# akanazawa/human_dynamics

Measured on NVIDIA H100. Metric: frames/sec (ResNet->f_movie->SMPL LBS), higher is better.
Workload: dtype f32 (wgmma 3x fp16 head/remainder split, fp32 two-level accumulate)

## Files before the change

human_dynamics_b200/csrc/conv_tc.cu:

```cuda
#include <cuda.h>
#include <cuda_fp16.h>
#include <cstdlib>
#include "conv_common.cuh"
#include "tc_ptx.cuh"

namespace hd {
namespace {

constexpr int BM = 128;
constexpr int A_TILE_BYTES = BM * 128;
constexpr int BOX_BYTES = 64 * 128;
constexpr int W_PROD = 8;
constexpr int STAGE_OUT = 1, STAGE_PAIR = 2;

using namespace ptx;

template <bool HALF, bool ASPLIT, int BN, bool RES = false>
struct Cfg {
  static_assert(BN == 64 || (BN == 128 && HALF && ASPLIT), "128-wide N tiles: pre-split fp16 path only");
  static_assert(!RES || ASPLIT, "residual by TMA: pre-split fp16 path only");
  static constexpr int PROD_THREADS = BN == 128 ? 128 : 256;
  static constexpr int NUM_THREADS = 256 + PROD_THREADS;
  static constexpr int ROW_STEP = PROD_THREADS / 8;
  static constexpr int ROWS = BM / ROW_STEP;
  static constexpr int PROD_REGS = BN == 128 ? 40 : 104, CONS_REGS = BN == 128 ? 232 : 152;
  static_assert(256 * CONS_REGS + PROD_THREADS * PROD_REGS <= 65536, "setmaxnreg split beyond the register file");
  static constexpr int NACC = BN / 2;
  static constexpr int STAGES = BN == 128 ? (RES ? 2 : 3) : (RES ? 3 : 4);
  static constexpr int BKE = HALF ? 64 : 32;
  static constexpr int B_TILE_BYTES = BN * 128;
  static constexpr int STAGE_BYTES = 2 * A_TILE_BYTES + 2 * B_TILE_BYTES;
  static constexpr int RES_OFFSET = STAGES * STAGE_BYTES;
  static constexpr int RES_SLOT_BYTES = RES ? 64 * BN * 4 : 0;
  static constexpr int STG_OFFSET = RES_OFFSET + 2 * RES_SLOT_BYTES;
  static constexpr int STG_BYTES = ASPLIT ? 2 * BOX_BYTES : 0;
  static constexpr int BAR_OFFSET = STG_OFFSET + 2 * STG_BYTES;
  static constexpr int SMEM_BYTES = BAR_OFFSET + 128 + 1024;
  static_assert(SMEM_BYTES <= 232448, "dynamic shared memory beyond the 227 KB a CTA can opt into");
  static constexpr int PF = HALF ? 2 : 3;
  static constexpr int V = HALF ? 2 : 1;
};

template <int R>
struct RowState {
  int n[R], iy[R], ix[R];
};

template <bool SPLIT, int PCH, bool HALF, bool GATHER, bool ASPLIT, int BN, bool RES>
__global__ void __launch_bounds__((Cfg<HALF, ASPLIT, BN, RES>::NUM_THREADS), 1)
conv_gemm_tc_kernel(const ConvParams p, const __grid_constant__ CUtensorMap tmap_hi, const __grid_constant__ CUtensorMap tmap_lo,
                    const __grid_constant__ CUtensorMap tmap_res, const __grid_constant__ CUtensorMap tmap_out,
                    const __grid_constant__ CUtensorMap tmap_out_hi, const __grid_constant__ CUtensorMap tmap_out_lo, const int stage) {
  using C = Cfg<HALF, ASPLIT, BN, RES>;
  constexpr int BKE = C::BKE, PF = C::PF, V = C::V, STAGES = C::STAGES, R = C::ROWS, RS = C::ROW_STEP, NA = C::NACC;
  extern __shared__ uint8_t smem_raw[];
  const uint32_t smem_base = (smem_u32(smem_raw) + 1023u) & ~1023u;
  uint8_t *smem = smem_raw + (smem_base - smem_u32(smem_raw));
  const uint32_t bar_base = smem_base + C::BAR_OFFSET;
  auto full_bar = [&](int s) { return bar_base + 8u * s; };
  auto empty_bar = [&](int s) { return bar_base + 8u * (STAGES + s); };
  auto res_bar = [&](int g) { return bar_base + 8u * (2 * STAGES + g); };

  const int warp = threadIdx.x >> 5, lane = threadIdx.x & 31;
  const int num_k = (GATHER ? p.K_pad : p.K) / BKE;
  const int tiles_n = (p.Cout + BN - 1) / BN;
  const int num_tiles = ((p.M + BM - 1) / BM) * tiles_n;
  const int my_tiles = (num_tiles - (int)blockIdx.x + (int)gridDim.x - 1) / (int)gridDim.x;

  if (threadIdx.x == 0) {
    for (int s = 0; s < STAGES; ++s) {
      mbar_init(full_bar(s), ASPLIT ? C::PROD_THREADS + 1 : 9);
      mbar_init(empty_bar(s), 8);
    }
    if (RES) for (int g = 0; g < 2; ++g) mbar_init(res_bar(g), 1);
    asm volatile("fence.mbarrier_init.release.cluster;" ::: "memory");
  }
  __syncthreads();
  const int xmode = p.dbg ? (int)p.dbg[15] : 0;

  if (warp >= W_PROD) {
    asm volatile("setmaxnreg.dec.sync.aligned.u32 %0;" ::"n"(C::PROD_REGS));
    const int t = threadIdx.x - W_PROD * 32;
    const int j = t & 7;
    const int rb = t >> 3;
    const uint32_t sw_off = (uint32_t)((j ^ (rb & 7)) << 4);
    const bool prof = p.dbg != nullptr && blockIdx.x == 0 && t == 0;
    long long t_wait = 0, t_start = prof && BN == 64 ? clock64() : 0;
    if (BN == 128 && prof) p.dbg[0] = clock64();
    const int total = my_tiles * num_k;
    auto load_b = [&](int s, int ti, int kc) {
      if (t != 0) return;
      const int n0 = (((int)blockIdx.x + ti * (int)gridDim.x) % tiles_n) * BN;
      const uint32_t b_hi = smem_base + s * C::STAGE_BYTES + 2 * A_TILE_BYTES;
      if (xmode & 2) { mbar_arrive(full_bar(s)); return; }
      const int boxes = (BN == 128 && n0 + 64 < p.Cout) ? 2 : 1;
      mbar_arrive_expect_tx(full_bar(s), (SPLIT ? 2 : 1) * boxes * BOX_BYTES);
      for (int b = 0; b < boxes; ++b) {
        tma_load_2d(b_hi + b * BOX_BYTES, &tmap_hi, full_bar(s), kc * BKE, n0 + 64 * b);
        if (SPLIT) tma_load_2d(b_hi + C::B_TILE_BYTES + b * BOX_BYTES, &tmap_lo, full_bar(s), kc * BKE, n0 + 64 * b);
      }
    };

    auto enter_tile = [&](int ti, RowState<R> &rs) {
      const int tile = (int)blockIdx.x + ti * (int)gridDim.x;
      const int m0 = (tile / tiles_n) * BM;
      const int hw = p.Ho * p.Wo;
#pragma unroll
      for (int i = 0; i < R; ++i) {
        const int m = m0 + rb + RS * i;
        if (m < p.M) {
          const int n = m / hw;
          const int r = m - n * hw;
          const int oy = r / p.Wo, ox = r - oy * p.Wo;
          rs.n[i] = n; rs.iy[i] = oy * p.stride - p.pad_t; rs.ix[i] = ox * p.stride - p.pad_l;
        } else {
          rs.n[i] = -1; rs.iy[i] = 0; rs.ix[i] = 0;
        }
      }
    };
    if constexpr (ASPLIT) {
      const __half *ihi = reinterpret_cast<const __half *>(p.in_hi);
      const __half *ilo = reinterpret_cast<const __half *>(p.in_lo);
      if (!p.planes && p.KH * p.KW <= 32 && (long long)p.n_img * p.H * p.W * p.in_ld < (1ll << 31)) {
        const uint32_t off0 = (uint32_t)rb * 128u + sw_off;
        int base[R];
        uint32_t mask[R];
        int kc = 0, ti = 0, tap = 0, ci0 = 0, kx = 0, ky = 0, tap_off = 0;
        for (int q = 0; q < total; ++q) {
          if (kc == 0) {
            const int tile = (int)blockIdx.x + ti * (int)gridDim.x;
            const int m0 = (tile / tiles_n) * BM + rb;
            const int hw = p.Ho * p.Wo;
#pragma unroll
            for (int i = 0; i < R; ++i) {
              const int m = m0 + RS * i;
              uint32_t mk = 0;
              int b = 0;
              if (m < p.M) {
                const int n = m / hw;
                const int r = m - n * hw;
                const int oy = r / p.Wo, ox = r - oy * p.Wo;
                const int iy0 = oy * p.stride - p.pad_t, ix0 = ox * p.stride - p.pad_l;
                b = ((n * p.H + iy0) * p.W + ix0) * p.in_ld + j * 8;
                int t = 0;
                for (int yy = 0; yy < p.KH; ++yy)
                  for (int xx = 0; xx < p.KW; ++xx, ++t)
                    if ((unsigned)(iy0 + yy) < (unsigned)p.H && (unsigned)(ix0 + xx) < (unsigned)p.W) mk |= 1u << t;
              }
              base[i] = b;
              mask[i] = mk;
            }
            tap = 0; ci0 = 0; kx = 0; ky = 0; tap_off = 0;
          }
          const int s = q % STAGES;
          const uint32_t ph = (uint32_t)(q / STAGES) & 1u;
          long long tw0 = prof ? clock64() : 0;
          mbar_wait(empty_bar(s), ph ^ 1u);
          if (prof) t_wait += clock64() - tw0;
          load_b(s, ti, kc);
          const uint32_t a_hi = smem_base + s * C::STAGE_BYTES + off0;
          const int eo = tap_off + ci0;
#pragma unroll
          for (int i = 0; i < R; ++i) {
            const bool ok = (mask[i] >> tap) & 1u;
            const int e = ok ? base[i] + eo : 0;
            cp_async16(a_hi + i * RS * 128, ihi + e, ok ? 16u : 0u);
            cp_async16(a_hi + A_TILE_BYTES + i * RS * 128, ilo + e, ok ? 16u : 0u);
          }
          asm volatile("cp.async.mbarrier.arrive.noinc.shared::cta.b64 [%0];" ::"r"(full_bar(s)) : "memory");
          ci0 += BKE;
          if (ci0 == p.Cin) {
            ci0 = 0; ++tap;
            if (++kx == p.KW) { kx = 0; ++ky; }
            tap_off = (ky * p.W + kx) * p.in_ld;
          }
          if (++kc == num_k) { kc = 0; ++ti; }
        }
      } else if (p.planes && (long long)p.n_img * p.H * p.W * p.in_ld < (1ll << 31)) {
        const uint32_t off0 = (uint32_t)rb * 128u + sw_off;
        const int jt = j >> 2;
        const int row_step = 2 * p.W * (int)p.in_ld;
        int base[R];
        int kc = 0, ti = 0;
        for (int q = 0; q < total; ++q) {
          if (kc == 0) {
            const int tile = (int)blockIdx.x + ti * (int)gridDim.x;
            const int m0 = (tile / tiles_n) * BM + rb;
            const int hw = p.Ho * p.Wo;
#pragma unroll
            for (int i = 0; i < R; ++i) {
              const int m = m0 + RS * i;
              int b = -1;
              if (m < p.M) {
                const int n = m / hw;
                const int r = m - n * hw;
                const int oy = r / p.Wo, ox = r - oy * p.Wo;
                b = ((n * p.H + oy * p.stride + jt) * p.W + ox * p.stride) * (int)p.in_ld + (j & 3) * 8;
              }
              base[i] = b;
            }
          }
          const int s = q % STAGES;
          const uint32_t ph = (uint32_t)(q / STAGES) & 1u;
          long long tw0 = prof ? clock64() : 0;
          mbar_wait(empty_bar(s), ph ^ 1u);
          if (prof) t_wait += clock64() - tw0;
          load_b(s, ti, kc);
          const uint32_t a_hi = smem_base + s * C::STAGE_BYTES + off0;
          const bool tap_ok = 2 * kc + jt < 7;
          const int eo = kc * row_step;
#pragma unroll
          for (int i = 0; i < R; ++i) {
            const bool ok = tap_ok && base[i] >= 0;
            const int e = ok ? base[i] + eo : 0;
            cp_async16_ca(a_hi + i * RS * 128, ihi + e, ok ? 16u : 0u);
            cp_async16_ca(a_hi + A_TILE_BYTES + i * RS * 128, ilo + e, ok ? 16u : 0u);
          }
          asm volatile("cp.async.mbarrier.arrive.noinc.shared::cta.b64 [%0];" ::"r"(full_bar(s)) : "memory");
          if (++kc == num_k) { kc = 0; ++ti; }
        }
      } else {
      RowState<R> rs;
      int kc = 0, ti = 0;
      for (int q = 0; q < total; ++q) {
        if (kc == 0) enter_tile(ti, rs);
        const int s = q % STAGES;
        const uint32_t ph = (uint32_t)(q / STAGES) & 1u;
        long long tw0 = prof ? clock64() : 0;
        mbar_wait(empty_bar(s), ph ^ 1u);
        if (prof) t_wait += clock64() - tw0;
        load_b(s, ti, kc);
        const int kb = kc * BKE;
        const int tap = p.planes ? 2 * kc + (j >> 2) : kb / p.Cin;
        const int ci = p.planes ? (j & 3) * 8 : kb - tap * p.Cin + j * 8;
        const int ky = tap / p.KW, kx = tap - ky * p.KW;
        const bool tap_ok = !p.planes || tap < 7;
        const uint32_t a_hi = smem_base + s * C::STAGE_BYTES, a_lo = a_hi + A_TILE_BYTES;
#pragma unroll
        for (int i = 0; i < R; ++i) {
          const int iy = rs.iy[i] + ky, ix = rs.ix[i] + kx;
          const bool ok = tap_ok && rs.n[i] >= 0 && iy >= 0 && iy < p.H && ix >= 0 && ix < p.W;
          const size_t e = ok ? ((size_t)((size_t)rs.n[i] * p.H + iy) * p.W + ix) * p.in_ld + ci : 0;
          const uint32_t off = (uint32_t)(rb + RS * i) * 128u + sw_off;
          if (p.planes) {
            cp_async16_ca(a_hi + off, ihi + e, ok ? 16u : 0u);
            cp_async16_ca(a_lo + off, ilo + e, ok ? 16u : 0u);
          } else {
            cp_async16(a_hi + off, ihi + e, ok ? 16u : 0u);
            cp_async16(a_lo + off, ilo + e, ok ? 16u : 0u);
          }
        }
        asm volatile("cp.async.mbarrier.arrive.noinc.shared::cta.b64 [%0];" ::"r"(full_bar(s)) : "memory");
        if (++kc == num_k) { kc = 0; ++ti; }
      }
      }
      cp_async_commit();
      cp_async_wait<0>();
      if (prof) { p.dbg[0] = clock64() - (BN == 128 ? p.dbg[0] : t_start); p.dbg[1] = t_wait; }
    } else {
    RowState<R> pf_rs, st_rs;
    float4 ring[PF][4 * V];
    uint32_t vmask[PF];
    int pf_kc = 0, pf_ti = 0;
    auto prefetch = [&](float4 *dst, uint32_t &vm) {
      if (pf_kc == 0) enter_tile(pf_ti, pf_rs);
      if (GATHER) {
        const int seg = p.KW * p.Cin, segp = (seg + 7) & ~7;
        const int g8 = (pf_kc * BKE + j * (4 * V)) / 8;
        const int gpr = segp >> 3;
        const int ky = g8 / gpr, r0 = (g8 - ky * gpr) * 8;
        vm = 0;
#pragma unroll
        for (int i = 0; i < 4; ++i) {
          const int iy = pf_rs.iy[i] + ky;
          const bool okr = pf_rs.n[i] >= 0 && ky < p.KH && iy >= 0 && iy < p.H;
          const int c0 = pf_rs.ix[i] * p.Cin + r0;
          const float *src = p.in + ((size_t)((size_t)(okr ? pf_rs.n[i] : 0) * p.H + (okr ? iy : 0)) * p.W) * p.in_ld + c0;
          const int rowlen = p.W * p.Cin;
          float xs[8];
#pragma unroll
          for (int e = 0; e < 8; ++e) {
            const bool ok = okr && (r0 + e) < seg && (c0 + e) >= 0 && (c0 + e) < rowlen;
            xs[e] = ok ? __ldg(src + e) : 0.f;
          }
          dst[i * V] = make_float4(xs[0], xs[1], xs[2], xs[3]);
          dst[i * V + V - 1] = make_float4(xs[4], xs[5], xs[6], xs[7]);
          if (pf_rs.n[i] >= 0) vm |= 1u << i;
        }
        if (++pf_kc == num_k) { pf_kc = 0; ++pf_ti; }
        return;
      }
      const int kb = pf_kc * BKE;
      const int tap = kb / p.Cin, ci = kb - tap * p.Cin + j * (4 * V);
      const int ky = tap / p.KW, kx = tap - ky * p.KW;
      vm = 0;
#pragma unroll
      for (int i = 0; i < 4; ++i) {
        const int iy = pf_rs.iy[i] + ky, ix = pf_rs.ix[i] + kx;
        const bool ok = pf_rs.n[i] >= 0 && iy >= 0 && iy < p.H && ix >= 0 && ix < p.W;
        if (ok && !(xmode & 4)) {
          const float4 *src = reinterpret_cast<const float4 *>(p.in + ((size_t)((size_t)pf_rs.n[i] * p.H + iy) * p.W + ix) * p.in_ld + ci);
#pragma unroll
          for (int v = 0; v < V; ++v) dst[i * V + v] = __ldg(src + v);
          vm |= 1u << i;
        } else {
#pragma unroll
          for (int v = 0; v < V; ++v) dst[i * V + v] = make_float4(0.f, 0.f, 0.f, 0.f);
        }
      }
      if (++pf_kc == num_k) { pf_kc = 0; ++pf_ti; }
    };
// ... 22 lines not shown
#pragma unroll
          for (int v = 0; v < V; ++v) {
            const float4 sc = __ldg(reinterpret_cast<const float4 *>(p.pre_scale + po) + v);
            const float4 sh = __ldg(reinterpret_cast<const float4 *>(p.pre_shift + po) + v);
            xs[4 * v] = xs[4 * v] * sc.x + sh.x; xs[4 * v + 1] = xs[4 * v + 1] * sc.y + sh.y;
            xs[4 * v + 2] = xs[4 * v + 2] * sc.z + sh.z; xs[4 * v + 3] = xs[4 * v + 3] * sc.w + sh.w;
          }
          if (p.pre_relu) {
#pragma unroll
            for (int e = 0; e < 4 * V; ++e) xs[e] = fmaxf(xs[e], 0.f);
          }
        }
        uint32_t h[4], l[4];
        if (!HALF) {
#pragma unroll
          for (int e = 0; e < 4; ++e) {
            const float hf = rn_tf32(xs[e]);
            h[e] = __float_as_uint(hf);
            l[e] = __float_as_uint(rn_tf32(xs[e] - hf));
          }
        } else {
#pragma unroll
          for (int e = 0; e < 4; ++e) split_f16x2(xs[2 * e], xs[2 * e + 1], h[e], l[e]);
        }
        const uint32_t off = (uint32_t)(rb + 32 * i) * 128u + sw_off;
        if (xmode & 1) continue;
        *reinterpret_cast<uint4 *>(a_hi + off) = make_uint4(h[0], h[1], h[2], h[3]);
        if (SPLIT) *reinterpret_cast<uint4 *>(a_lo + off) = make_uint4(l[0], l[1], l[2], l[3]);
      }
      asm volatile("fence.proxy.async.shared::cta;" ::: "memory");
      __syncwarp();
      if (lane == 0) mbar_arrive(full_bar(s));
      if (++st_kc == num_k) { st_kc = 0; ++st_ti; }
    };
#pragma unroll
    for (int u = 0; u < PF - 1; ++u)
      if (u < total) prefetch(ring[u], vmask[u]);
    for (int q0 = 0; q0 < total; q0 += PF) {
#pragma unroll
      for (int u = 0; u < PF; ++u) {
        const int q = q0 + u;
        if (q < total) {
          if (q + PF - 1 < total) prefetch(ring[(u + PF - 1) % PF], vmask[(u + PF - 1) % PF]);
          consume(q, ring[u], vmask[u]);
        }
      }
    }
    if (prof) { p.dbg[0] = clock64() - t_start; p.dbg[1] = t_wait; }
    }
  } else if (warp < W_PROD) {
    asm volatile("setmaxnreg.inc.sync.aligned.u32 %0;" ::"n"(C::CONS_REGS));
    const int wg = warp >> 2;
    const bool prof = p.dbg != nullptr && blockIdx.x == 0 && threadIdx.x == 0;
    long long t_wait = 0, t_start = prof && BN == 64 && !RES ? clock64() : 0;
    if ((RES || BN == 128) && prof) p.dbg[2] = clock64();
    if (prof) { p.dbg[3] = 0; p.dbg[4] = 0; p.dbg[5] = 0; p.dbg[6] = 0; }
    const int hw = p.Ho * p.Wo;
    const int frow = wg * 64 + (warp & 3) * 16 + (lane >> 2);
    const int fcol = 2 * (lane & 3);
    float acc[NA], accx[NA], sums[NA];
#pragma unroll
    for (int i = 0; i < NA; ++i) { acc[i] = 0.f; accx[i] = 0.f; }
    uint8_t *res_sm = smem + C::RES_OFFSET + wg * C::RES_SLOT_BYTES;
    const bool res_issuer = RES && (threadIdx.x & 127) == 0;
    const bool stg_issuer = ASPLIT && (threadIdx.x & 127) == 0;
    auto load_res = [&](int ti) {
      const int tile = (int)blockIdx.x + ti * (int)gridDim.x;
      const int r0 = (tile / tiles_n) * BM + 64 * wg, c0 = (tile % tiles_n) * BN;
      const int cols = p.Cout - c0 < BN ? p.Cout - c0 : BN;
      const int boxes = r0 < p.M ? (cols + 31) / 32 : 0;
      const uint32_t slot = smem_base + C::RES_OFFSET + wg * C::RES_SLOT_BYTES;
      mbar_arrive_expect_tx(res_bar(wg), boxes * (64 * 128));
      for (int b = 0; b < boxes; ++b) tma_load_2d(slot + b * (64 * 128), &tmap_res, res_bar(wg), c0 + 32 * b, r0);
    };
    if (res_issuer && my_tiles > 0) load_res(0);
    int q = 0;
    for (int ti = 0; ti < my_tiles; ++ti) {
#pragma unroll
      for (int i = 0; i < NA; ++i) sums[i] = 0.f;
      for (int kc = 0; kc < num_k; ++kc, ++q) {
        const int s = q % STAGES;
        const uint32_t ph = (uint32_t)(q / STAGES) & 1u;
        const bool group_start = (kc % PCH) == 0;
        if (BN == 128 && prof) p.dbg[3] -= clock64();
        const long long tw0 = BN == 64 && prof ? clock64() : 0;
        mbar_wait(full_bar(s), ph);
        if (BN == 64 && prof) t_wait += clock64() - tw0;
        if (BN == 128 && prof) p.dbg[3] += clock64();
        if (ASPLIT) asm volatile("fence.proxy.async.shared::cta;" ::: "memory");
        const uint32_t a_hi = smem_base + s * C::STAGE_BYTES + wg * (64 * 128);
        const uint32_t a_lo = a_hi + A_TILE_BYTES;
        const uint32_t b_hi = smem_base + s * C::STAGE_BYTES + 2 * A_TILE_BYTES;
        const uint32_t b_lo = b_hi + C::B_TILE_BYTES;
        const uint64_t da_hi = make_smem_desc(a_hi), da_lo = make_smem_desc(a_lo);
        const uint64_t db_hi = make_smem_desc(b_hi), db_lo = make_smem_desc(b_lo);
        fence_regs(acc);
        if (SPLIT) fence_regs(accx);
        wgmma_fence();
#pragma unroll
        for (int k = 0; k < 4; ++k) {
          const uint64_t adv = (uint64_t)((k * 32) >> 4);
          if constexpr (BN == 128) {
            wgmma_m64n128k16_f16(accx, da_lo + adv, db_hi + adv, (kc | k) != 0);
            wgmma_m64n128k16_f16(accx, da_hi + adv, db_lo + adv, 1u);
            wgmma_m64n128k16_f16(acc, da_hi + adv, db_hi + adv, !(group_start && k == 0));
          } else if constexpr (HALF) {
            wgmma_m64n64k16_f16(accx, da_lo + adv, db_hi + adv, (kc | k) != 0);
            wgmma_m64n64k16_f16(accx, da_hi + adv, db_lo + adv, 1u);
            wgmma_m64n64k16_f16(acc, da_hi + adv, db_hi + adv, !(group_start && k == 0));
          } else {
            if (SPLIT) {
              wgmma_m64n64k8_tf32(accx, da_lo + adv, db_hi + adv, (kc | k) != 0);
              wgmma_m64n64k8_tf32(accx, da_hi + adv, db_lo + adv, 1u);
            }
            wgmma_m64n64k8_tf32(acc, da_hi + adv, db_hi + adv, !(group_start && k == 0));
          }
        }
        wgmma_commit();
        wgmma_wait<0>();
        fence_regs(acc);
        if (SPLIT) fence_regs(accx);
        __syncwarp();
        if (lane == 0) mbar_arrive(empty_bar(s));
        if ((kc % PCH) == PCH - 1 || kc == num_k - 1) {
#pragma unroll
          for (int i = 0; i < NA; ++i) sums[i] += acc[i];
        }
      }
      if (SPLIT) {
#pragma unroll
        for (int i = 0; i < NA; ++i) sums[i] += accx[i] * (HALF ? (1.0f / 2048.0f) : 1.0f);
      }
      if (prof) p.dbg[4] -= clock64();
      const int tile = (int)blockIdx.x + ti * (int)gridDim.x;
      const int m0 = (tile / tiles_n) * BM, n0 = (tile % tiles_n) * BN;
      if (RES && prof) p.dbg[5] -= clock64();
      if (RES) mbar_wait(res_bar(wg), (uint32_t)ti & 1u);
      if (RES && prof) p.dbg[5] += clock64();
      auto row_geom = [&](int m, int &n_img, int &oy, int &ox) {
        n_img = 0; oy = 0; ox = 0;
        if (p.out_sub || (!RES && p.res && !(p.res_stride == 1 && p.res_H == p.Ho && p.res_W == p.Wo))) {
          n_img = m / hw;
          const int r = m - n_img * hw;
          oy = r / p.Wo; ox = r - oy * p.Wo;
        }
      };
      auto res_row = [&](int m, int n_img, int oy, int ox) -> const float * {
        if (RES || !p.res) return nullptr;
        const size_t rr = (p.res_stride == 1 && p.res_H == p.Ho && p.res_W == p.Wo)
                              ? (size_t)m
                              : ((size_t)n_img * p.res_H + (size_t)oy * p.res_stride) * p.res_W + (size_t)ox * p.res_stride;
        return p.res + rr * p.res_ld;
      };
      auto out_row = [&](int m, int n_img, int oy, int ox) -> float * {
        if (!p.out) return nullptr;
        if (!p.out_sub) return p.out + (size_t)m * p.out_ld;
        if (oy % p.out_sub != 0 || ox % p.out_sub != 0) return nullptr;
        const int Hs = (p.Ho + p.out_sub - 1) / p.out_sub, Ws = (p.Wo + p.out_sub - 1) / p.out_sub;
        return p.out + ((size_t)((size_t)n_img * Hs + oy / p.out_sub) * Ws + ox / p.out_sub) * p.out_ld;
      };
      auto value2 = [&](int c, const float2 *rs, const float *rrow, float &y0, float &y1) {
        if (p.post_scale) { const float2 sc = __ldg(reinterpret_cast<const float2 *>(p.post_scale + c)); y0 *= sc.x; y1 *= sc.y; }
        if (p.post_shift) { const float2 sh = __ldg(reinterpret_cast<const float2 *>(p.post_shift + c)); y0 += sh.x; y1 += sh.y; }
        if (RES) { const float2 r = *rs; y0 += r.x; y1 += r.y; }
        else if (rrow) { const float2 r = *reinterpret_cast<const float2 *>(rrow + c); y0 += r.x; y1 += r.y; }
        if (p.post_relu) { y0 = fmaxf(y0, 0.f); y1 = fmaxf(y1, 0.f); }
      };
      auto pair2 = [&](int c, float a0, float a1, uint32_t &hh, uint32_t &ll) {
        if (p.post2_scale) { const float2 sc = __ldg(reinterpret_cast<const float2 *>(p.post2_scale + c)); a0 *= sc.x; a1 *= sc.y; }
        if (p.post2_shift) { const float2 sh = __ldg(reinterpret_cast<const float2 *>(p.post2_shift + c)); a0 += sh.x; a1 += sh.y; }
        if (p.post2_relu) { a0 = fmaxf(a0, 0.f); a1 = fmaxf(a1, 0.f); }
        split_f16x2(a0, a1, hh, ll);
      };
      if constexpr (ASPLIT) {
        const bool st32 = (stage & STAGE_OUT) != 0, st2 = (stage & STAGE_PAIR) != 0;
        uint8_t *stg = smem + C::STG_OFFSET + wg * C::STG_BYTES;
        const uint32_t stg_a = smem_base + C::STG_OFFSET + wg * C::STG_BYTES;
        const int r0 = m0 + 64 * wg;
        const uint32_t rsw = (uint32_t)(lane >> 2);
        auto acquire = [&](bool after_out) {
// ... 20 lines not shown
              if (c0 + 8 * jj + fcol >= p.Cout) continue;
              const uint32_t piece = (uint32_t)(2 * (jj & 3) + ((lane & 3) >> 1)) ^ rsw;
              const float2 sc = vsc ? __ldg(reinterpret_cast<const float2 *>(vsc + 8 * jj)) : make_float2(0.f, 0.f);
              const float2 sh = vsh ? __ldg(reinterpret_cast<const float2 *>(vsh + 8 * jj)) : make_float2(0.f, 0.f);
#pragma unroll
              for (int h = 0; h < 2; ++h) {
                if (!rok[h]) continue;
                float2 *f32 = reinterpret_cast<float2 *>(brow + h * 1024 + (jj >> 2) * BOX_BYTES + piece * 16);
                float y0 = sums[4 * j + 2 * h], y1 = sums[4 * j + 2 * h + 1];
                if (vsc) { y0 = __fmul_rn(y0, sc.x); y1 = __fmul_rn(y1, sc.y); }
                if (vsh) { y0 = __fadd_rn(y0, sh.x); y1 = __fadd_rn(y1, sh.y); }
                if (RES) { const float2 r = *f32; y0 = __fadd_rn(y0, r.x); y1 = __fadd_rn(y1, r.y); }
                if (p.post_relu) { y0 = fmaxf(y0, 0.f); y1 = fmaxf(y1, 0.f); }
                *f32 = make_float2(y0, y1);
                sums[4 * j + 2 * h] = y0; sums[4 * j + 2 * h + 1] = y1;
              }
            }
          } else {
#pragma unroll
          for (int h = 0; h < 2; ++h) {
            const int m = m0 + frow + 8 * h;
            if (m >= p.M) continue;
            int n_img, oy, ox;
            row_geom(m, n_img, oy, ox);
            const float *rrow = res_row(m, n_img, oy, ox);
            float *orow = st32 ? nullptr : out_row(m, n_img, oy, ox);
            uint8_t *brow = (RES ? res_sm + 2 * cc * BOX_BYTES : stg) + (frow - 64 * wg + 8 * h) * 128 + 8 * (lane & 1);
#pragma unroll
            for (int jj = 0; jj < 8; ++jj) {
              const int j = 8 * cc + jj;
              const int c = n0 + 8 * j + fcol;
              if (c >= p.Cout) continue;
              const uint32_t piece = (uint32_t)(2 * (jj & 3) + ((lane & 3) >> 1)) ^ rsw;
              float2 *f32 = reinterpret_cast<float2 *>(brow + (jj >> 2) * BOX_BYTES + piece * 16);
              float y0 = sums[4 * j + 2 * h], y1 = sums[4 * j + 2 * h + 1];
              value2(c, f32, rrow, y0, y1);
              if (st32) *f32 = make_float2(y0, y1);
              else if (orow) *reinterpret_cast<float2 *>(orow + c) = make_float2(y0, y1);
              sums[4 * j + 2 * h] = y0; sums[4 * j + 2 * h + 1] = y1;
            }
          }
          }
          if (st32) {
            fence_proxy_async();
            named_bar_sync(3 + wg, 128);
            if (issue) {
              const uint32_t src = RES ? smem_base + C::RES_OFFSET + wg * C::RES_SLOT_BYTES + 2 * cc * BOX_BYTES : stg_a;
              tma_store_2d(&tmap_out, src, c0, r0);
              if (c0 + 32 < p.Cout) tma_store_2d(&tmap_out, src + BOX_BYTES, c0 + 32, r0);
            }
            if (stg_issuer) bulk_commit();
          }
          if (p.out_hi) {
            if (st2) acquire(RES && st32);
            if (st2) {
              uint8_t *brow = stg + (frow - 64 * wg) * 128 + 4 * (lane & 3);
              const float *vsc = p.post2_scale ? p.post2_scale + c0 + fcol : nullptr, *vsh = p.post2_shift ? p.post2_shift + c0 + fcol : nullptr;
#pragma unroll
              for (int jj = 0; jj < 8; ++jj) {
                const int j = 8 * cc + jj;
                if (c0 + 8 * jj + fcol >= p.Cout) continue;
                const float2 sc = vsc ? __ldg(reinterpret_cast<const float2 *>(vsc + 8 * jj)) : make_float2(0.f, 0.f);
                const float2 sh = vsh ? __ldg(reinterpret_cast<const float2 *>(vsh + 8 * jj)) : make_float2(0.f, 0.f);
#pragma unroll
                for (int h = 0; h < 2; ++h) {
                  if (!rok[h]) continue;
                  float a0 = sums[4 * j + 2 * h], a1 = sums[4 * j + 2 * h + 1];
                  if (vsc) { a0 = __fmul_rn(a0, sc.x); a1 = __fmul_rn(a1, sc.y); }
                  if (vsh) { a0 = __fadd_rn(a0, sh.x); a1 = __fadd_rn(a1, sh.y); }
                  if (p.post2_relu) { a0 = fmaxf(a0, 0.f); a1 = fmaxf(a1, 0.f); }
                  uint32_t hh, ll;
                  split_f16x2(a0, a1, hh, ll);
                  uint32_t *hs = reinterpret_cast<uint32_t *>(brow + h * 1024 + (((uint32_t)jj ^ rsw) * 16));
                  hs[0] = hh;
                  hs[BOX_BYTES / 4] = ll;
                }
              }
            } else {
#pragma unroll
            for (int h = 0; h < 2; ++h) {
              const int m = m0 + frow + 8 * h;
              if (m >= p.M) continue;
              __half *hrow = reinterpret_cast<__half *>(p.out_hi) + (size_t)m * p.out2_ld;
              __half *lrow = reinterpret_cast<__half *>(p.out_lo) + (size_t)m * p.out2_ld;
              uint8_t *brow = stg + (frow - 64 * wg + 8 * h) * 128 + 4 * (lane & 3);
#pragma unroll
              for (int jj = 0; jj < 8; ++jj) {
                const int j = 8 * cc + jj;
                const int c = n0 + 8 * j + fcol;
                if (c >= p.Cout) continue;
                uint32_t hh, ll;
                pair2(c, sums[4 * j + 2 * h], sums[4 * j + 2 * h + 1], hh, ll);
                if (st2) {
                  uint32_t *hs = reinterpret_cast<uint32_t *>(brow + (((uint32_t)jj ^ rsw) * 16));
                  hs[0] = hh;
                  hs[BOX_BYTES / 4] = ll;
                } else {
                  *reinterpret_cast<uint32_t *>(hrow + c) = hh;
                  *reinterpret_cast<uint32_t *>(lrow + c) = ll;
                }
              }
            }
            }
            if (st2) {
              fence_proxy_async();
              named_bar_sync(3 + wg, 128);
              if (issue) {
                tma_store_2d(&tmap_out_hi, stg_a, c0, r0);
                tma_store_2d(&tmap_out_lo, stg_a + BOX_BYTES, c0, r0);
              }
              if (stg_issuer) bulk_commit();
            }
          }
        }
      } else {
#pragma unroll
      for (int h = 0; h < 2; ++h) {
        const int m = m0 + frow + 8 * h;
        if (m >= p.M) continue;
        int n_img, oy, ox;
        row_geom(m, n_img, oy, ox);
        const float *rrow = res_row(m, n_img, oy, ox);
        float *orow = out_row(m, n_img, oy, ox);
        __half *hrow = p.out_hi ? reinterpret_cast<__half *>(p.out_hi) + (size_t)m * p.out2_ld : nullptr;
        __half *lrow = p.out_hi ? reinterpret_cast<__half *>(p.out_lo) + (size_t)m * p.out2_ld : nullptr;
#pragma unroll
        for (int j = 0; j < BN / 8; ++j) {
          const int c = n0 + 8 * j + fcol;
          if (c >= p.Cout) continue;
          const bool two = c + 1 < p.Cout;
          float y[2] = {sums[4 * j + 2 * h], sums[4 * j + 2 * h + 1]};
          if (p.vec_out) {
            value2(c, nullptr, rrow, y[0], y[1]);
            if (orow) *reinterpret_cast<float2 *>(orow + c) = make_float2(y[0], y[1]);
            if (hrow) {
              uint32_t hh, ll;
              pair2(c, y[0], y[1], hh, ll);
              *reinterpret_cast<uint32_t *>(hrow + c) = hh;
              *reinterpret_cast<uint32_t *>(lrow + c) = ll;
            }
          } else {
#pragma unroll
            for (int e = 0; e < 2; ++e) {
              if (e == 1 && !two) break;
              float v = y[e];
              if (p.post_scale) v *= __ldg(p.post_scale + c + e);
              if (p.post_shift) v += __ldg(p.post_shift + c + e);
              if (rrow) v += rrow[c + e];
              if (p.post_relu) v = fmaxf(v, 0.f);
              if (orow) orow[c + e] = v;
            }
          }
        }
      }
      }
      if (RES && ti + 1 < my_tiles) {
        if (prof) p.dbg[6] -= clock64();
        named_bar_sync(1 + wg, 128);
        if (res_issuer) {
          if (stage & STAGE_OUT) {
            if (stage & STAGE_PAIR) bulk_wait_read<1>();
            else bulk_wait_read<0>();
          }
          load_res(ti + 1);
        }
        if (prof) p.dbg[6] += clock64();
      }
      if (prof) p.dbg[4] += clock64();
    }
    if (stg_issuer) bulk_wait_all();
    if (prof) { p.dbg[2] = clock64() - (RES || BN == 128 ? p.dbg[2] : t_start); if (BN == 64) p.dbg[3] = t_wait; }
  }
}

typedef CUresult (*EncodeTiledFn)(CUtensorMap *, CUtensorMapDataType, cuuint32_t, void *, const cuuint64_t *, const cuuint64_t *,
                                  const cuuint32_t *, const cuuint32_t *, CUtensorMapInterleave, CUtensorMapSwizzle,
                                  CUtensorMapL2promotion, CUtensorMapFloatOOBfill);

EncodeTiledFn get_encode_fn() {
  static EncodeTiledFn fn = nullptr;
  static bool tried = false;
  if (!tried) {
    tried = true;
    void *ptr = nullptr;
    cudaDriverEntryPointQueryResult qres;
    cudaError_t e = cudaGetDriverEntryPoint("cuTensorMapEncodeTiled", &ptr, cudaEnableDefault, &qres);
    if (e == cudaSuccess && qres == cudaDriverEntryPointSuccess) fn = reinterpret_cast<EncodeTiledFn>(ptr);
    else (void)cudaGetLastError();
  }
  return fn;
}

constexpr int kMaxDevices = 64;

int encode_epilogue_map(CUtensorMap *tm, bool fp16, const void *base, int cols, int rows, long long ld_bytes, const char *what) {
  EncodeTiledFn fn = get_encode_fn();
  if (!fn) { set_last_error_text("cuTensorMapEncodeTiled unavailable (no CUDA driver?)"); return HD_ERR_UNSUPPORTED; }
  const cuuint64_t gdim[2] = {(cuuint64_t)cols, (cuuint64_t)rows};
  const cuuint64_t gstride[1] = {(cuuint64_t)ld_bytes};
  const cuuint32_t box[2] = {fp16 ? 64u : 32u, 64u};
  const cuuint32_t estr[2] = {1u, 1u};
  CUresult r = fn(tm, fp16 ? CU_TENSOR_MAP_DATA_TYPE_FLOAT16 : CU_TENSOR_MAP_DATA_TYPE_FLOAT32, 2, const_cast<void *>(base), gdim, gstride,
                  box, estr, CU_TENSOR_MAP_INTERLEAVE_NONE, CU_TENSOR_MAP_SWIZZLE_128B, CU_TENSOR_MAP_L2_PROMOTION_L2_128B,
                  CU_TENSOR_MAP_FLOAT_OOB_FILL_NONE);
  if (r != CUDA_SUCCESS) {
    char msg[96];
    snprintf(msg, sizeof(msg), "cuTensorMapEncodeTiled (%s) failed with CUresult %d", what, (int)r);
    set_last_error_text(msg);
    return HD_ERR_CUDA;
  }
  return HD_OK;
}

template <bool SPLIT, int PCH, bool HALF, bool GATHER = false, bool ASPLIT = false, int BN = 64, bool RES = false>
int launch_tc(const ConvParams &p, const hd_conv_desc *d, cudaStream_t st) {
  using C = Cfg<HALF, ASPLIT, BN, RES>;
  static bool configured[kMaxDevices] = {};
  static int num_sms[kMaxDevices] = {};
  int dev = 0;
  cudaGetDevice(&dev);
  if (dev < 0 || dev >= kMaxDevices) { set_last_error_text("conv_gemm_tc: device ordinal out of range"); return HD_ERR_UNSUPPORTED; }
  if (!configured[dev]) {
    cudaError_t e = cudaFuncSetAttribute(conv_gemm_tc_kernel<SPLIT, PCH, HALF, GATHER, ASPLIT, BN, RES>,
                                         cudaFuncAttributeMaxDynamicSharedMemorySize, C::SMEM_BYTES);
    if (e != cudaSuccess) { set_last_error("conv_gemm_tc attr", e); return HD_ERR_CUDA; }
    cudaDeviceGetAttribute(&num_sms[dev], cudaDevAttrMultiProcessorCount, dev);
    if (num_sms[dev] <= 0) { set_last_error_text("conv_gemm_tc: no multiprocessor count"); return HD_ERR_CUDA; }
    configured[dev] = true;
  }
  alignas(64) CUtensorMap thi, tlo;
  const void *mhi = d->tmap_hi_n64 ? d->tmap_hi_n64 : d->tmap_hi;
  const void *mlo = d->tmap_hi_n64 ? d->tmap_lo_n64 : d->tmap_lo;
  memcpy(&thi, mhi, sizeof(CUtensorMap));
  memcpy(&tlo, mlo ? mlo : mhi, sizeof(CUtensorMap));
  alignas(64) CUtensorMap tres, tout, tohi, tolo;
  memcpy(&tres, &thi, sizeof(CUtensorMap));
  memcpy(&tout, &thi, sizeof(CUtensorMap));
  memcpy(&tohi, &thi, sizeof(CUtensorMap));
  memcpy(&tolo, &thi, sizeof(CUtensorMap));
  int rc = HD_OK;
  if (RES) rc = encode_epilogue_map(&tres, false, p.res, p.Cout, p.M, p.res_ld * 4, "residual");
  int stage = 0;
  if (ASPLIT && p.out && !p.out_sub) {
    stage |= STAGE_OUT;
    if (rc == HD_OK) rc = encode_epilogue_map(&tout, false, p.out, p.Cout, p.M, p.out_ld * 4, "output");
  }
  if (ASPLIT && p.out_hi && p.out2_ld % 8 == 0) {
    stage |= STAGE_PAIR;
    if (rc == HD_OK) rc = encode_epilogue_map(&tohi, true, p.out_hi, p.Cout, p.M, p.out2_ld * 2, "output head");
    if (rc == HD_OK) rc = encode_epilogue_map(&tolo, true, p.out_lo, p.Cout, p.M, p.out2_ld * 2, "output remainder");
  }
  if (rc != HD_OK) return rc;
  const int num_tiles = ceil_div(p.M, BM) * ceil_div(p.Cout, BN);
  dim3 grid(num_tiles < num_sms[dev] ? num_tiles : num_sms[dev]);
  conv_gemm_tc_kernel<SPLIT, PCH, HALF, GATHER, ASPLIT, BN, RES>
      <<<grid, C::NUM_THREADS, C::SMEM_BYTES, st>>>(p, thi, tlo, tres, tout, tohi, tolo, stage);
  return check_launch("conv_gemm_tc_kernel");
}

bool wide_n_tile(const ConvParams &p) {
  if (p.Cout <= 64) return false;
  int dev = 0, sms = 0;
  cudaGetDevice(&dev);
  cudaDeviceGetAttribute(&sms, cudaDevAttrMultiProcessorCount, dev);
  if (sms <= 0) return true;
  const long long m_tiles = ceil_div(p.M, BM);
  const long long w128 = (m_tiles * ceil_div(p.Cout, 128) + sms - 1) / sms, w64 = (m_tiles * ceil_div(p.Cout, 64) + sms - 1) / sms;
  return 16 * w128 <= 9 * w64;
}

}

int launch_conv_tc(const ConvParams &p, const hd_conv_desc *d, cudaStream_t st) {
  const bool split_b = d->impl != HD_IMPL_TC_1XTF32;
  if (!d->tmap_hi || (split_b && !d->tmap_lo) || (!d->tmap_hi_n64 && d->tmap_lo_n64) || (d->tmap_hi_n64 && split_b && !d->tmap_lo_n64)) {
    set_last_error_text("hd_conv_gemm(tc): missing tensor maps (tmap_hi/tmap_lo, and tmap_hi_n64/tmap_lo_n64 together or not at all)");
    return HD_ERR_INVALID;
  }
  const bool half = d->impl == HD_IMPL_TC_3XF16;
  const int bke = half ? 64 : 32;
  if (p.out_sub) {
    const bool res_plain = !p.res || (p.res_stride == 1 && p.res_H == p.Ho && p.res_W == p.Wo);
    const bool maps = (!p.res || d->tmap_res) && (!p.out_hi || (d->tmap_out_hi && d->tmap_out_lo));
    if (!p.in_hi || p.planes || !maps || !res_plain || p.Cout % 32 != 0 || (d->flags & HD_CONV_NO_TMA_EPILOGUE)) {
      set_last_error_text("hd_conv_gemm: out_subsample needs the activation-map epilogue (pre-split input, Cout % 32 == 0, activation maps given)");
      return HD_ERR_UNSUPPORTED;
    }
  }
  if ((p.out_hi || p.in_hi) && (!half || !p.vec_out)) {
    set_last_error_text("hd_conv_gemm(tc): pre-split activations need impl 3 and 16-byte aligned, 4-column-multiple outputs");
    return HD_ERR_INVALID;
  }
  if (p.in_hi && p.planes) {
    if (p.Cin != 32 || p.KH != 8 || p.KW != 1 || p.stride != 2 || p.pad_t != 0 || p.pad_l != 0 || p.in_ld != 4 || p.Cout > 64 ||
        p.W % 2 != 0 || 2 * (p.Wo - 1) + 8 > p.W || 2 * (p.Ho - 1) + 7 > p.H || !aligned16(p.in_hi) || !aligned16(p.in_lo) || p.pre_scale) {
      set_last_error_text("hd_conv_gemm(tc planes): needs the conv1 plane geometry (Cin 32, KH 8, KW 1, stride 2, in_ld 4, even W)");
      return HD_ERR_INVALID;
    }
    return launch_tc<true, 2, true, false, true>(p, d, st);
  }
  if (p.in_hi) {
    if (p.Cin % 64 != 0 || p.K % 64 != 0 || p.in_ld % 8 != 0 || !aligned16(p.in_hi) || !aligned16(p.in_lo) || p.pre_scale) {
      set_last_error_text("hd_conv_gemm(tc split-A): needs Cin % 64 == 0, in_ld % 8 == 0, aligned in_hi/in_lo, no prologue");
      return HD_ERR_INVALID;
    }
    const bool res_rows = p.res && p.res_stride == 1 && p.res_H == p.Ho && p.res_W == p.Wo && p.K <= 8 * 64;
    if (wide_n_tile(p))
      return res_rows ? launch_tc<true, 2, true, false, true, 128, true>(p, d, st) : launch_tc<true, 2, true, false, true, 128>(p, d, st);
    return res_rows ? launch_tc<true, 2, true, false, true, 64, true>(p, d, st) : launch_tc<true, 2, true, false, true>(p, d, st);
  }
  if (half && p.Cin % bke != 0) {
    const int segp = (p.KW * p.Cin + 7) & ~7;
    if (p.K_pad % 64 != 0 || p.K_pad < p.KH * segp || p.Cout > 64 || p.pre_scale || p.in_ld != p.Cin) {
      set_last_error_text("hd_conv_gemm(tc gather): needs K_pad % 64 == 0, K_pad >= KH*roundup8(KW*Cin), Cout <= 64, dense pixels, no prologue");
      return HD_ERR_INVALID;
    }
    return launch_tc<true, 2, true, true>(p, d, st);
  }
  if (!p.in || p.Cin % bke != 0 || p.in_ld % 4 != 0 || !aligned16(p.in) || p.K % bke != 0 ||
      (p.pre_scale && (!aligned16(p.pre_scale) || !aligned16(p.pre_shift) || p.pre_img_stride % 4 != 0))) {
    set_last_error_text("hd_conv_gemm(tc): needs Cin % 32 (tf32) / % 64 (fp16) == 0 and 16-byte aligned input / prologue vectors");
    return HD_ERR_INVALID;
  }
  if (half) return launch_tc<true, 2, true>(p, d, st);
  return d->impl != HD_IMPL_TC_1XTF32 ? launch_tc<true, 2, false>(p, d, st) : launch_tc<false, 8, false>(p, d, st);
}

}

extern "C" int hd_make_weight_tmap(const void *w_nk, int rows, int k_pad, int box_rows, int elem_bytes, void *tmap_out) {
  HD_REQUIRE(w_nk && tmap_out && rows > 0 && k_pad > 0 && (elem_bytes == 4 || elem_bytes == 2) && k_pad % (128 / elem_bytes) == 0 &&
                 box_rows == 64 && rows % box_rows == 0 && hd::aligned16(w_nk),
             "hd_make_weight_tmap: bad arguments");
  hd::EncodeTiledFn fn = hd::get_encode_fn();
  if (!fn) { hd::set_last_error_text("cuTensorMapEncodeTiled unavailable (no CUDA driver?)"); return HD_ERR_UNSUPPORTED; }
  alignas(64) CUtensorMap tm;
  const cuuint64_t gdim[2] = {(cuuint64_t)k_pad, (cuuint64_t)rows};
  const cuuint64_t gstride[1] = {(cuuint64_t)k_pad * (cuuint64_t)elem_bytes};
  const cuuint32_t box[2] = {(cuuint32_t)(128 / elem_bytes), (cuuint32_t)box_rows};
  const cuuint32_t estr[2] = {1u, 1u};
  CUresult r = fn(&tm, elem_bytes == 4 ? CU_TENSOR_MAP_DATA_TYPE_FLOAT32 : CU_TENSOR_MAP_DATA_TYPE_FLOAT16, 2, const_cast<void *>(w_nk),
                  gdim, gstride, box, estr, CU_TENSOR_MAP_INTERLEAVE_NONE, CU_TENSOR_MAP_SWIZZLE_128B,
                  CU_TENSOR_MAP_L2_PROMOTION_L2_128B, CU_TENSOR_MAP_FLOAT_OOB_FILL_NONE);
  if (r != CUDA_SUCCESS) {
    char msg[96];
    snprintf(msg, sizeof(msg), "cuTensorMapEncodeTiled failed with CUresult %d", (int)r);
    hd::set_last_error_text(msg);
    return HD_ERR_CUDA;
  }
  memcpy(tmap_out, &tm, sizeof(tm));
  return HD_OK;
}

extern "C" int hd_make_act_tmap(const void *base, long long rows, int cols, long long ld_elems, int elem_bytes, void *tmap_out) {
  HD_REQUIRE(base && tmap_out && rows > 0 && cols > 0 && ld_elems >= cols && (elem_bytes == 4 || elem_bytes == 2) && hd::aligned16(base) &&
                 (ld_elems * elem_bytes) % 16 == 0,
             "hd_make_act_tmap: bad arguments (16-byte aligned base and row pitch required)");
  hd::EncodeTiledFn fn = hd::get_encode_fn();
  if (!fn) { hd::set_last_error_text("cuTensorMapEncodeTiled unavailable (no CUDA driver?)"); return HD_ERR_UNSUPPORTED; }
// ... 18 lines not shown
```

Baseline: 12920.

## Add two-CTA-per-SM variant for short-K 1x1 pre-split convolutions

```diff
diff --git a/human_dynamics_b200/csrc/conv_tc.cu b/human_dynamics_b200/csrc/conv_tc.cu
--- a/human_dynamics_b200/csrc/conv_tc.cu
+++ b/human_dynamics_b200/csrc/conv_tc.cu
@@ -15,28 +15,32 @@
 
 using namespace ptx;
 
-template <bool HALF, bool ASPLIT, int BN, bool RES = false>
+template <bool HALF, bool ASPLIT, int BN, bool RES = false, bool SHORT = false>
 struct Cfg {
   static_assert(BN == 64 || (BN == 128 && HALF && ASPLIT), "128-wide N tiles: pre-split fp16 path only");
   static_assert(!RES || ASPLIT, "residual by TMA: pre-split fp16 path only");
-  static constexpr int PROD_THREADS = BN == 128 ? 128 : 256;
+  static_assert(!SHORT || (BN == 64 && HALF && ASPLIT), "two CTAs per SM: 64-wide pre-split fp16 tiles only");
+  static constexpr int CTAS = SHORT ? 2 : 1;
+  static constexpr int PROD_THREADS = BN == 128 || SHORT ? 128 : 256;
   static constexpr int NUM_THREADS = 256 + PROD_THREADS;
   static constexpr int ROW_STEP = PROD_THREADS / 8;
   static constexpr int ROWS = BM / ROW_STEP;
-  static constexpr int PROD_REGS = BN == 128 ? 40 : 104, CONS_REGS = BN == 128 ? 232 : 152;
-  static_assert(256 * CONS_REGS + PROD_THREADS * PROD_REGS <= 65536, "setmaxnreg split beyond the register file");
+  static constexpr int PROD_REGS = SHORT ? 32 : BN == 128 ? 40 : 104, CONS_REGS = SHORT ? 104 : BN == 128 ? 232 : 152;
+  static_assert(CTAS * (256 * CONS_REGS + PROD_THREADS * PROD_REGS) <= 65536, "setmaxnreg split beyond the register file");
   static constexpr int NACC = BN / 2;
-  static constexpr int STAGES = BN == 128 ? (RES ? 2 : 3) : (RES ? 3 : 4);
+  static constexpr int STAGES = SHORT ? 1 : BN == 128 ? (RES ? 2 : 3) : (RES ? 3 : 4);
   static constexpr int BKE = HALF ? 64 : 32;
   static constexpr int B_TILE_BYTES = BN * 128;
   static constexpr int STAGE_BYTES = 2 * A_TILE_BYTES + 2 * B_TILE_BYTES;
   static constexpr int RES_OFFSET = STAGES * STAGE_BYTES;
-  static constexpr int RES_SLOT_BYTES = RES ? 64 * BN * 4 : 0;
-  static constexpr int STG_OFFSET = RES_OFFSET + 2 * RES_SLOT_BYTES;
+  static constexpr int RES_SLOT_BYTES = RES || SHORT ? 64 * BN * 4 : 0;
+  static constexpr int STG_OFFSET = SHORT ? RES_OFFSET : RES_OFFSET + 2 * RES_SLOT_BYTES;
   static constexpr int STG_BYTES = ASPLIT ? 2 * BOX_BYTES : 0;
-  static constexpr int BAR_OFFSET = STG_OFFSET + 2 * STG_BYTES;
+  static_assert(!SHORT || STG_BYTES == RES_SLOT_BYTES, "SHORT: the staging buffer is the residual slot");
+  static constexpr int BAR_OFFSET = SHORT ? RES_OFFSET + 2 * RES_SLOT_BYTES : STG_OFFSET + 2 * STG_BYTES;
   static constexpr int SMEM_BYTES = BAR_OFFSET + 128 + 1024;
   static_assert(SMEM_BYTES <= 232448, "dynamic shared memory beyond the 227 KB a CTA can opt into");
+  static_assert(CTAS * (SMEM_BYTES + 1024) <= 233472, "CTAS CTAs (and the 1 KB each reserves) beyond an SM's 228 KB");
   static constexpr int PF = HALF ? 2 : 3;
   static constexpr int V = HALF ? 2 : 1;
 };
@@ -46,12 +50,13 @@
   int n[R], iy[R], ix[R];
 };
 
-template <bool SPLIT, int PCH, bool HALF, bool GATHER, bool ASPLIT, int BN, bool RES>
-__global__ void __launch_bounds__((Cfg<HALF, ASPLIT, BN, RES>::NUM_THREADS), 1)
+template <bool SPLIT, int PCH, bool HALF, bool GATHER, bool ASPLIT, int BN, bool RES, bool SHORT>
+__global__ void __launch_bounds__((Cfg<HALF, ASPLIT, BN, RES, SHORT>::NUM_THREADS), (Cfg<HALF, ASPLIT, BN, RES, SHORT>::CTAS))
 conv_gemm_tc_kernel(const ConvParams p, const __grid_constant__ CUtensorMap tmap_hi, const __grid_constant__ CUtensorMap tmap_lo,
                     const __grid_constant__ CUtensorMap tmap_res, const __grid_constant__ CUtensorMap tmap_out,
                     const __grid_constant__ CUtensorMap tmap_out_hi, const __grid_constant__ CUtensorMap tmap_out_lo, const int stage) {
-  using C = Cfg<HALF, ASPLIT, BN, RES>;
+  using C = Cfg<HALF, ASPLIT, BN, RES, SHORT>;
+  constexpr bool MEM_STAMPS = BN == 128 || SHORT;
   constexpr int BKE = C::BKE, PF = C::PF, V = C::V, STAGES = C::STAGES, R = C::ROWS, RS = C::ROW_STEP, NA = C::NACC;
   extern __shared__ uint8_t smem_raw[];
   const uint32_t smem_base = (smem_u32(smem_raw) + 1023u) & ~1023u;
@@ -85,8 +90,15 @@
     const int rb = t >> 3;
     const uint32_t sw_off = (uint32_t)((j ^ (rb & 7)) << 4);
     const bool prof = p.dbg != nullptr && blockIdx.x == 0 && t == 0;
-    long long t_wait = 0, t_start = prof && BN == 64 ? clock64() : 0;
-    if (BN == 128 && prof) p.dbg[0] = clock64();
+    long long t_wait = 0, t_start = prof && !MEM_STAMPS ? clock64() : 0;
+    if (MEM_STAMPS && prof) { p.dbg[0] = clock64(); p.dbg[1] = 0; }
+    auto wait_empty = [&](int s, uint32_t ph) {
+      if (MEM_STAMPS && prof) p.dbg[1] -= clock64();
+      const long long tw0 = !MEM_STAMPS && prof ? clock64() : 0;
+      mbar_wait(empty_bar(s), ph ^ 1u);
+      if (!MEM_STAMPS && prof) t_wait += clock64() - tw0;
+      if (MEM_STAMPS && prof) p.dbg[1] += clock64();
+    };
     const int total = my_tiles * num_k;
     auto load_b = [&](int s, int ti, int kc) {
       if (t != 0) return;
@@ -121,7 +133,7 @@
     if constexpr (ASPLIT) {
       const __half *ihi = reinterpret_cast<const __half *>(p.in_hi);
       const __half *ilo = reinterpret_cast<const __half *>(p.in_lo);
-      if (!p.planes && p.KH * p.KW <= 32 && (long long)p.n_img * p.H * p.W * p.in_ld < (1ll << 31)) {
+      if (SHORT || (!p.planes && p.KH * p.KW <= 32 && (long long)p.n_img * p.H * p.W * p.in_ld < (1ll << 31))) {
         const uint32_t off0 = (uint32_t)rb * 128u + sw_off;
         int base[R];
         uint32_t mask[R];
@@ -147,22 +159,20 @@
                   for (int xx = 0; xx < p.KW; ++xx, ++t)
                     if ((unsigned)(iy0 + yy) < (unsigned)p.H && (unsigned)(ix0 + xx) < (unsigned)p.W) mk |= 1u << t;
               }
-              base[i] = b;
+              base[i] = SHORT && !(mk & 1u) ? -1 : b;
               mask[i] = mk;
             }
             tap = 0; ci0 = 0; kx = 0; ky = 0; tap_off = 0;
           }
           const int s = q % STAGES;
           const uint32_t ph = (uint32_t)(q / STAGES) & 1u;
-          long long tw0 = prof ? clock64() : 0;
-          mbar_wait(empty_bar(s), ph ^ 1u);
-          if (prof) t_wait += clock64() - tw0;
+          wait_empty(s, ph);
           load_b(s, ti, kc);
           const uint32_t a_hi = smem_base + s * C::STAGE_BYTES + off0;
-          const int eo = tap_off + ci0;
+          const int eo = SHORT ? ci0 : tap_off + ci0;
 #pragma unroll
           for (int i = 0; i < R; ++i) {
-            const bool ok = (mask[i] >> tap) & 1u;
+            const bool ok = SHORT ? base[i] >= 0 : (mask[i] >> tap) & 1u;
             const int e = ok ? base[i] + eo : 0;
             cp_async16(a_hi + i * RS * 128, ihi + e, ok ? 16u : 0u);
             cp_async16(a_hi + A_TILE_BYTES + i * RS * 128, ilo + e, ok ? 16u : 0u);
@@ -176,7 +186,7 @@
           }
           if (++kc == num_k) { kc = 0; ++ti; }
         }
-      } else if (p.planes && (long long)p.n_img * p.H * p.W * p.in_ld < (1ll << 31)) {
+      } else if (!SHORT && p.planes && (long long)p.n_img * p.H * p.W * p.in_ld < (1ll << 31)) {
         const uint32_t off0 = (uint32_t)rb * 128u + sw_off;
         const int jt = j >> 2;
         const int row_step = 2 * p.W * (int)p.in_ld;
@@ -202,9 +212,7 @@
           }
           const int s = q % STAGES;
           const uint32_t ph = (uint32_t)(q / STAGES) & 1u;
-          long long tw0 = prof ? clock64() : 0;
-          mbar_wait(empty_bar(s), ph ^ 1u);
-          if (prof) t_wait += clock64() - tw0;
+          wait_empty(s, ph);
           load_b(s, ti, kc);
           const uint32_t a_hi = smem_base + s * C::STAGE_BYTES + off0;
           const bool tap_ok = 2 * kc + jt < 7;
@@ -219,16 +227,14 @@
           asm volatile("cp.async.mbarrier.arrive.noinc.shared::cta.b64 [%0];" ::"r"(full_bar(s)) : "memory");
           if (++kc == num_k) { kc = 0; ++ti; }
         }
-      } else {
+      } else if (!SHORT) {
       RowState<R> rs;
       int kc = 0, ti = 0;
       for (int q = 0; q < total; ++q) {
         if (kc == 0) enter_tile(ti, rs);
         const int s = q % STAGES;
         const uint32_t ph = (uint32_t)(q / STAGES) & 1u;
-        long long tw0 = prof ? clock64() : 0;
-        mbar_wait(empty_bar(s), ph ^ 1u);
-        if (prof) t_wait += clock64() - tw0;
+        wait_empty(s, ph);
         load_b(s, ti, kc);
         const int kb = kc * BKE;
         const int tap = p.planes ? 2 * kc + (j >> 2) : kb / p.Cin;
@@ -256,7 +262,7 @@
       }
       cp_async_commit();
       cp_async_wait<0>();
-      if (prof) { p.dbg[0] = clock64() - (BN == 128 ? p.dbg[0] : t_start); p.dbg[1] = t_wait; }
+      if (prof) { p.dbg[0] = clock64() - (MEM_STAMPS ? p.dbg[0] : t_start); if (!MEM_STAMPS) p.dbg[1] = t_wait; }
     } else {
     RowState<R> pf_rs, st_rs;
     float4 ring[PF][4 * V];
@@ -385,13 +391,14 @@
     asm volatile("setmaxnreg.inc.sync.aligned.u32 %0;" ::"n"(C::CONS_REGS));
     const int wg = warp >> 2;
     const bool prof = p.dbg != nullptr && blockIdx.x == 0 && threadIdx.x == 0;
-    long long t_wait = 0, t_start = prof && BN == 64 && !RES ? clock64() : 0;
-    if ((RES || BN == 128) && prof) p.dbg[2] = clock64();
+    long long t_wait = 0, t_start = prof && !MEM_STAMPS && !RES ? clock64() : 0;
+    if ((RES || MEM_STAMPS) && prof) p.dbg[2] = clock64();
     if (prof) { p.dbg[3] = 0; p.dbg[4] = 0; p.dbg[5] = 0; p.dbg[6] = 0; }
     const int hw = p.Ho * p.Wo;
     const int frow = wg * 64 + (warp & 3) * 16 + (lane >> 2);
     const int fcol = 2 * (lane & 3);
-    float acc[NA], accx[NA], sums[NA];
+    float acc[NA], accx[NA], sums_[SHORT ? 1 : NA];
+    float *const sums = SHORT ? acc : sums_;
 #pragma unroll
     for (int i = 0; i < NA; ++i) { acc[i] = 0.f; accx[i] = 0.f; }
     uint8_t *res_sm = smem + C::RES_OFFSET + wg * C::RES_SLOT_BYTES;
@@ -409,17 +416,19 @@
     if (res_issuer && my_tiles > 0) load_res(0);
     int q = 0;
     for (int ti = 0; ti < my_tiles; ++ti) {
-#pragma unroll
-      for (int i = 0; i < NA; ++i) sums[i] = 0.f;
+      if (!SHORT) {
+#pragma unroll
+        for (int i = 0; i < NA; ++i) sums[i] = 0.f;
+      }
       for (int kc = 0; kc < num_k; ++kc, ++q) {
         const int s = q % STAGES;
         const uint32_t ph = (uint32_t)(q / STAGES) & 1u;
         const bool group_start = (kc % PCH) == 0;
-        if (BN == 128 && prof) p.dbg[3] -= clock64();
-        const long long tw0 = BN == 64 && prof ? clock64() : 0;
+        if (MEM_STAMPS && prof) p.dbg[3] -= clock64();
+        const long long tw0 = !MEM_STAMPS && prof ? clock64() : 0;
         mbar_wait(full_bar(s), ph);
-        if (BN == 64 && prof) t_wait += clock64() - tw0;
-        if (BN == 128 && prof) p.dbg[3] += clock64();
+        if (!MEM_STAMPS && prof) t_wait += clock64() - tw0;
+        if (MEM_STAMPS && prof) p.dbg[3] += clock64();
         if (ASPLIT) asm volatile("fence.proxy.async.shared::cta;" ::: "memory");
         const uint32_t a_hi = smem_base + s * C::STAGE_BYTES + wg * (64 * 128);
         const uint32_t a_lo = a_hi + A_TILE_BYTES;
@@ -455,10 +464,14 @@
         if (SPLIT) fence_regs(accx);
         __syncwarp();
         if (lane == 0) mbar_arrive(empty_bar(s));
-        if ((kc % PCH) == PCH - 1 || kc == num_k - 1) {
+        if (!SHORT && ((kc % PCH) == PCH - 1 || kc == num_k - 1)) {
 #pragma unroll
           for (int i = 0; i < NA; ++i) sums[i] += acc[i];
         }
+      }
+      if (SHORT) {
+#pragma unroll
+        for (int i = 0; i < NA; ++i) acc[i] = __fadd_rn(0.f, acc[i]);
       }
       if (SPLIT) {
 #pragma unroll
@@ -585,7 +598,7 @@
             if (stg_issuer) bulk_commit();
           }
           if (p.out_hi) {
-            if (st2) acquire(RES && st32);
+            if (st2) acquire(RES && st32 && !SHORT);
             if (st2) {
               uint8_t *brow = stg + (frow - 64 * wg) * 128 + 4 * (lane & 3);
               const float *vsc = p.post2_scale ? p.post2_scale + c0 + fcol : nullptr, *vsh = p.post2_shift ? p.post2_shift + c0 + fcol : nullptr;
@@ -691,7 +704,9 @@
         if (prof) p.dbg[6] -= clock64();
         named_bar_sync(1 + wg, 128);
         if (res_issuer) {
-          if (stage & STAGE_OUT) {
+          if (SHORT) {
+            if (stage) bulk_wait_read<0>();
+          } else if (stage & STAGE_OUT) {
             if (stage & STAGE_PAIR) bulk_wait_read<1>();
             else bulk_wait_read<0>();
           }
@@ -702,7 +717,7 @@
       if (prof) p.dbg[4] += clock64();
     }
     if (stg_issuer) bulk_wait_all();
-    if (prof) { p.dbg[2] = clock64() - (RES || BN == 128 ? p.dbg[2] : t_start); if (BN == 64) p.dbg[3] = t_wait; }
+    if (prof) { p.dbg[2] = clock64() - (RES || MEM_STAMPS ? p.dbg[2] : t_start); if (!MEM_STAMPS) p.dbg[3] = t_wait; }
   }
 }
 
@@ -745,16 +760,16 @@
   return HD_OK;
 }
 
-template <bool SPLIT, int PCH, bool HALF, bool GATHER = false, bool ASPLIT = false, int BN = 64, bool RES = false>
+template <bool SPLIT, int PCH, bool HALF, bool GATHER = false, bool ASPLIT = false, int BN = 64, bool RES = false, bool SHORT = false>
 int launch_tc(const ConvParams &p, const hd_conv_desc *d, cudaStream_t st) {
-  using C = Cfg<HALF, ASPLIT, BN, RES>;
+  using C = Cfg<HALF, ASPLIT, BN, RES, SHORT>;
   static bool configured[kMaxDevices] = {};
   static int num_sms[kMaxDevices] = {};
   int dev = 0;
   cudaGetDevice(&dev);
   if (dev < 0 || dev >= kMaxDevices) { set_last_error_text("conv_gemm_tc: device ordinal out of range"); return HD_ERR_UNSUPPORTED; }
   if (!configured[dev]) {
-    cudaError_t e = cudaFuncSetAttribute(conv_gemm_tc_kernel<SPLIT, PCH, HALF, GATHER, ASPLIT, BN, RES>,
+    cudaError_t e = cudaFuncSetAttribute(conv_gemm_tc_kernel<SPLIT, PCH, HALF, GATHER, ASPLIT, BN, RES, SHORT>,
                                          cudaFuncAttributeMaxDynamicSharedMemorySize, C::SMEM_BYTES);
     if (e != cudaSuccess) { set_last_error("conv_gemm_tc attr", e); return HD_ERR_CUDA; }
     cudaDeviceGetAttribute(&num_sms[dev], cudaDevAttrMultiProcessorCount, dev);
@@ -785,8 +800,9 @@
   }
   if (rc != HD_OK) return rc;
   const int num_tiles = ceil_div(p.M, BM) * ceil_div(p.Cout, BN);
-  dim3 grid(num_tiles < num_sms[dev] ? num_tiles : num_sms[dev]);
-  conv_gemm_tc_kernel<SPLIT, PCH, HALF, GATHER, ASPLIT, BN, RES>
+  const int ctas = C::CTAS * num_sms[dev];
+  dim3 grid(num_tiles < ctas ? num_tiles : ctas);
+  conv_gemm_tc_kernel<SPLIT, PCH, HALF, GATHER, ASPLIT, BN, RES, SHORT>
       <<<grid, C::NUM_THREADS, C::SMEM_BYTES, st>>>(p, thi, tlo, tres, tout, tohi, tolo, stage);
   return check_launch("conv_gemm_tc_kernel");
 }
@@ -802,6 +818,26 @@
   return 16 * w128 <= 9 * w64;
 }
 
+template <bool RES>
+bool short_k_two_ctas() {
+  using C = Cfg<true, true, 64, RES, true>;
+  static int two[kMaxDevices] = {};
+  int dev = 0;
+  cudaGetDevice(&dev);
+  if (dev < 0 || dev >= kMaxDevices) return false;
+  if (two[dev] == 0) {
+    const auto kernel = conv_gemm_tc_kernel<true, 2, true, false, true, 64, RES, true>;
+    int n = 0;
+    if (cudaFuncSetAttribute(kernel, cudaFuncAttributeMaxDynamicSharedMemorySize, C::SMEM_BYTES) != cudaSuccess ||
+        cudaOccupancyMaxActiveBlocksPerMultiprocessor(&n, kernel, C::NUM_THREADS, C::SMEM_BYTES) != cudaSuccess) {
+      (void)cudaGetLastError();
+      n = 0;
+    }
+    two[dev] = n >= 2 ? 1 : -1;
+  }
+  return two[dev] > 0;
+}
+
 }
 
 int launch_conv_tc(const ConvParams &p, const hd_conv_desc *d, cudaStream_t st) {
@@ -838,6 +874,10 @@
       return HD_ERR_INVALID;
     }
     const bool res_rows = p.res && p.res_stride == 1 && p.res_H == p.Ho && p.res_W == p.Wo && p.K <= 8 * 64;
+    const bool short_k = p.K <= 2 * 64 && p.KH * p.KW == 1 && (long long)p.n_img * p.H * p.W * p.in_ld < (1ll << 31) &&
+                         (p.res ? res_rows : p.out_hi != nullptr);
+    if (short_k && (res_rows ? short_k_two_ctas<true>() : short_k_two_ctas<false>()))
+      return res_rows ? launch_tc<true, 2, true, false, true, 64, true, true>(p, d, st) : launch_tc<true, 2, true, false, true, 64, false, true>(p, d, st);
     if (wide_n_tile(p))
       return res_rows ? launch_tc<true, 2, true, false, true, 128, true>(p, d, st) : launch_tc<true, 2, true, false, true, 128>(p, d, st);
     return res_rows ? launch_tc<true, 2, true, false, true, 64, true>(p, d, st) : launch_tc<true, 2, true, false, true>(p, d, st);
```

After: 13570, median of 6. +5.1%, better.
